# iclavera/learning_to_adapt

Hardware: AMD Instinct MI355X
Metric: controller-steps/sec (n_cand=2000, H=30, ens=5) (higher is better)
Workload: dtype f32

## Files before the change

### learning_to_adapt_amd/csrc/l2a_mfma.h

```cpp
#pragma once

#include <type_traits>

#include "l2a_kernels.h"

#ifndef L2A_XEARLY
#define L2A_XEARLY 1
#endif

#ifndef L2A_NW
#define L2A_NW 4
#endif

typedef unsigned int u32x4 __attribute__((ext_vector_type(4)));
__device__ __forceinline__ __amdgpu_buffer_rsrc_t l2a_rsrc(const void* base, long long bytes) {
    return __builtin_amdgcn_make_buffer_rsrc(const_cast<void*>(base), 0, (int)bytes, 0x00020000);
}
__device__ __forceinline__ f32x4 l2a_ldw(__amdgpu_buffer_rsrc_t rs, int voff, int soff) {
    return __builtin_bit_cast(f32x4, __builtin_amdgcn_raw_buffer_load_b128(rs, voff, soff, 0));
}

template <bool GACT>
__device__ __forceinline__ f32x4 l2a_actv(f32x4 v, int kind, float floor) {
    if (GACT) return l2a_act4(v, kind);
    v.x = l2a_max_nan(v.x, floor); v.y = l2a_max_nan(v.y, floor);
    v.z = l2a_max_nan(v.z, floor); v.w = l2a_max_nan(v.w, floor);
    return v;
}

__device__ __forceinline__ float l2a_sum_xor16(float x) {
    const unsigned int u = __float_as_uint(x);
    const auto r = __builtin_amdgcn_permlane16_swap(u, u, false, false);
    return __uint_as_float(r[0]) + __uint_as_float(r[1]);
}
__device__ __forceinline__ float l2a_sum_xor32(float x) {
    const unsigned int u = __float_as_uint(x);
    const auto r = __builtin_amdgcn_permlane32_swap(u, u, false, false);
    return __uint_as_float(r[0]) + __uint_as_float(r[1]);
}

#define L2A_MFMA4(a, b, c) __builtin_amdgcn_mfma_f32_4x4x1f32((a), (b), (c), 0, 0, 0)

#define L2A_OPAQUE(v) asm volatile("" : "+v"(v))

#ifndef L2A_TIMELINE
#define L2A_TS(slot)
#else
#define L2A_TS(slot)                                                                        \
    if (p.dbg && pairid == 0 && e < 8 && grp < 2) {                                         \
        unsigned long long ts_;                                                             \
        asm volatile("s_memtime %0\n\ts_waitcnt lgkmcnt(0)" : "=s"(ts_) : : "memory");       \
        if (lane == 0) p.dbg[(((long long)(grp * p.h + t) * 8 + e) * 8 + wave) * 16 + (slot)] = ts_; \
    }
#endif

#define L2A_STAGE_MFMA(CA, CB)                                                             \
    _Pragma("unroll") for (int ii = 0; ii < 4; ++ii)                                       \
        _Pragma("unroll") for (int nt = 0; nt < NT; ++nt)                                  \
            _Pragma("unroll") for (int tt = TW - 1; tt >= 0; --tt)    \
                acc[nt][tt] = L2A_MFMA(CA[tt][ii], CB[nt][ii], acc[nt][tt]);

#define L2A_STAGE(CA, CB, FA, FB, SOFF, IMM, GF)                                           \
    {                                                                                      \
        _Pragma("unroll") for (int tt = 0; tt < TW; ++tt)                                  \
            FA[tt] = l2a_ldw(rs, voff[tt] + (IMM), (SOFF));                                \
        _Pragma("unroll") for (int nt = 0; nt < NT; ++nt)                                  \
            FB[nt] = hin[(nt * HT + (GF)) * 64 + lane];                                    \
        L2A_STAGE_MFMA(CA, CB)                                                             \
         \
        __builtin_amdgcn_sched_group_barrier(0x100, NT, 0);                                \
        _Pragma("unroll") for (int tt = 0; tt < TW; ++tt) {                                \
            __builtin_amdgcn_sched_group_barrier(0x008, 4 * NT, 0);                        \
            __builtin_amdgcn_sched_group_barrier(0x020, 1, 0);                             \
        }                                                                                  \
        __builtin_amdgcn_sched_barrier(0);                                                 \
    }

#define L2A_PFT_MAX 6
#define L2A_PFT(TW_, OT_) ((OT_) <= 2 ? ((TW_) < L2A_PFT_MAX ? (TW_) : L2A_PFT_MAX) : ((TW_) < 2 ? (TW_) : 2))

template <int NT, int TW, int TPW, int OT, bool LAST>
__device__ __forceinline__ void l2a_hidden_gemm(__amdgpu_buffer_rsrc_t rs, __amdgpu_buffer_rsrc_t rsn,
                                                const int (&voff)[TPW], const int (&voffn)[TPW], int twn,
                                                int tile0, const f32x4* hin,
                                                f32x4 (&aA)[TPW], f32x4 (&aB)[TPW],
                                                f32x4 (&pfO)[TPW][OT], f32x4 (&acc)[NT][TPW], int lane,
                                                const float* bias_lds, f32x4 (&bias)[TPW], const int (&olane)[OT]) {
    constexpr int HT = L2A_NW * TPW;
    static_assert(HT % 4 == 0, "the k-group pipeline is unrolled by 4");
    f32x4 aC[TW], aD[TW], bA[NT], bB[NT], bC[NT], bD[NT];
#pragma unroll
    for (int nt = 0; nt < NT; ++nt) {
        bA[nt] = hin[(nt * HT + 0) * 64 + lane];
        bB[nt] = hin[(nt * HT + 1) * 64 + lane];
#pragma unroll
        for (int tt = 0; tt < TW; ++tt) acc[nt][tt] = (f32x4){0.f, 0.f, 0.f, 0.f};
    }
#pragma unroll
    for (int nt = 0; nt < NT; ++nt) { L2A_OPAQUE(bA[nt]); L2A_OPAQUE(bB[nt]); }
    __builtin_amdgcn_sched_barrier(0);

#pragma unroll 1
    for (int g = 0; g < HT - 4; g += 4) {
        const int soff = (g + 2) * 1024;
        L2A_STAGE(aA, bA, aC, bC, soff, 0, g + 2)
        L2A_STAGE(aB, bB, aD, bD, soff, 1024, g + 3)
        L2A_STAGE(aC, bC, aA, bA, soff, 2048, g + 4)
        L2A_STAGE(aD, bD, aB, bB, soff, 3072, g + 5)
    }
    L2A_STAGE(aA, bA, aC, bC, (HT - 2) * 1024, 0, HT - 2)
    L2A_STAGE(aB, bB, aD, bD, (HT - 2) * 1024, 1024, HT - 1)
    {
        if (LAST) {
#pragma unroll
            for (int tt = 0; tt < L2A_PFT(TW, OT); ++tt)
#pragma unroll
                for (int c = 0; c < OT; ++c)
                    if (((tt * OT + c) & 1) == 0)
                        pfO[tt][c] = l2a_ldw(rsn, olane[c] + (tile0 + tt) * 1024, c * HT * 1024);
        } else {
#pragma unroll
            for (int tt = 0; tt < TPW; ++tt)
                if (tt < twn) aA[tt] = l2a_ldw(rsn, voffn[tt], 0);
        }
        L2A_STAGE_MFMA(aC, bC)
        __builtin_amdgcn_sched_barrier(0);
    }
    {
#pragma unroll
        for (int tt = 0; tt < TW; ++tt) bias[tt] = *reinterpret_cast<const f32x4*>(bias_lds + 16 * tt);
        if (LAST) {
#pragma unroll
            for (int tt = 0; tt < L2A_PFT(TW, OT); ++tt)
#pragma unroll
                for (int c = 0; c < OT; ++c)
                    if (((tt * OT + c) & 1) == 1)
                        pfO[tt][c] = l2a_ldw(rsn, olane[c] + (tile0 + tt) * 1024, c * HT * 1024);
        } else {
#pragma unroll
            for (int tt = 0; tt < TPW; ++tt)
                if (tt < twn) aB[tt] = l2a_ldw(rsn, voffn[tt] + 1024, 0);
        }
        L2A_STAGE_MFMA(aD, bD)
        __builtin_amdgcn_sched_barrier(0);
    }
}

template <int NT, int TW, int TPW, int OT, int NPF, bool O4, class PF>
__device__ __forceinline__ void l2a_out_phase(const f32x4 (&hreg)[NT][TPW], f32x4 (&pfO)[TPW][OT],
                                              __amdgpu_buffer_rsrc_t rs_out, int tile0, PF prefetch,
                                              f32x4* pbuf, int chunk0, int lane, const int (&olane)[OT]) {
    constexpr int HT = L2A_NW * TPW;
    constexpr int CS = TPW / 2;
    constexpr int NCH = TW / CS;
    f32x4 a[TW][OT];
#pragma unroll
    for (int tt = 0; tt < TW; ++tt)
#pragma unroll
        for (int c = 0; c < OT; ++c)
            a[tt][c] = (tt < L2A_PFT(TW, OT)) ? pfO[tt][c]
                                              : l2a_ldw(rs_out, olane[c] + (tile0 + tt) * 1024, c * HT * 1024);
    prefetch();
    f32x4 acc[NCH][NT][OT];
#pragma unroll
    for (int ch = 0; ch < NCH; ++ch)
#pragma unroll
        for (int nt = 0; nt < NT; ++nt)
#pragma unroll
            for (int c = 0; c < OT; ++c) acc[ch][nt][c] = (f32x4){0.f, 0.f, 0.f, 0.f};
#pragma unroll
    for (int t2 = 0; t2 < CS; ++t2)
#pragma unroll
        for (int ii = 0; ii < 4; ++ii)
#pragma unroll
            for (int ch = 0; ch < NCH; ++ch)
#pragma unroll
                for (int nt = 0; nt < NT; ++nt)
#pragma unroll
                    for (int c = 0; c < OT; ++c)
                        acc[ch][nt][c] = (O4 && c == OT - 1)
                            ? L2A_MFMA4(a[ch * CS + t2][c][ii], hreg[nt][ch * CS + t2][ii], acc[ch][nt][c])
                            : L2A_MFMA(a[ch * CS + t2][c][ii], hreg[nt][ch * CS + t2][ii], acc[ch][nt][c]);
    {
        constexpr int NLATE = (TW - L2A_PFT(TW, OT)) * OT;
        constexpr int NMFMA = TW * 4 * NT * OT;
#pragma unroll
        for (int i = 0; i < NLATE; ++i) {
            __builtin_amdgcn_sched_group_barrier(0x020, 1, 0);
            __builtin_amdgcn_sched_group_barrier(0x008, 2, 0);
        }
        constexpr int PER = (NMFMA - 2 * NLATE) / NPF > 0 ? (NMFMA - 2 * NLATE) / NPF : 1;
#pragma unroll
        for (int i = 0; i < NPF; ++i) {
            __builtin_amdgcn_sched_group_barrier(0x008, PER, 0);
            __builtin_amdgcn_sched_group_barrier(0x020, 1, 0);
        }
    }
#pragma unroll
    for (int nt = 0; nt < NT; ++nt)
#pragma unroll
        for (int c = 0; c < OT; ++c)
            pbuf[((chunk0 * NT + nt) * OT + c) * 64 + lane] = (NCH == 2) ? acc[0][nt][c] + acc[NCH - 1][nt][c] : acc[0][nt][c];
}

template <int NT, int TPW, int OT, int KG0, bool GACT, int K0L = 4, bool N1 = false, bool O4 = false, bool FAN = false, bool WHOLE = false>
__global__ void __launch_bounds__(64 * L2A_NW) l2a_rollout_mfma_k(const L2AKParams p) {
    static_assert(!(FAN && WHOLE), "an instance is general, member fan or whole-tiles-only");
    constexpr bool NOHALF = FAN || WHOLE;
    constexpr int HT = L2A_NW * TPW;
    constexpr int TH = TPW / 2;
    static_assert(TPW % 2 == 0, "half members split a wave's tiles in two");
    constexpr int CST_BOUT = 32 * KG0 + 32 * OT;
    constexpr int CST_BHID = CST_BOUT + 16 * OT;
    constexpr int PS = L2A_NW * NT * OT * 64;
    const int NRM_SET = p.cst_set;
    const int LB = p.lb;
    extern __shared__ __attribute__((aligned(16))) char l2a_smem[];
    f32x4* buf0 = reinterpret_cast<f32x4*>(l2a_smem);
    f32x4* buf1 = buf0 + p.sa_elems;
    f32x4* pbase = buf0 + (LB > 1 ? LB : 2) * p.sa_elems;
    float* nrm = reinterpret_cast<float*>(buf0 + p.cst_off);

    const int tid = threadIdx.x;
    const int lane = tid & 63;
    const int wave = __builtin_amdgcn_readfirstlane(tid >> 6);
    const int jc = lane & 15;
    const int qq = lane >> 4;
    const int c0 = wave * TPW;
    int olane[OT];
#pragma unroll
    for (int c = 0; c < OT; ++c) olane[c] = ((O4 && c == OT - 1) ? ((lane & 48) | (lane & 3)) : lane) * 16;

    const int tail = p.split_from >= 0;
    const int in_tail = tail && (int)blockIdx.x >= p.split_from;
    const int split = FAN ? 3 : WHOLE ? 0 : (tail ? (in_tail ? p.split : 0) : p.split);
    const int n_tiles = p.m * p.tiles_per_env;
    const int n_pairs = tail ? n_tiles - p.split_from : n_tiles;
    int bid, grp, lpair, pairid;
    if (!tail && p.pl_units > 0) {
        const int hx = (int)blockIdx.x & 7, idx = (int)blockIdx.x >> 3;
        const int xcd = hx;
        const int f = p.pl_f, wide = p.pl_r * (f + 1);
        int u, k, xu;
        if (xcd < wide) { u = xcd / (f + 1); k = xcd - u * (f + 1); xu = f + 1; }
// ... 60 lines not shown
        float v;
        if (o < CST_BOUT) v = src[p.nm_off + o];
        else if (o < CST_BHID) v = src[p.pk_bout + (o - CST_BOUT)];
        else {
            const int l = (o - CST_BHID) / (16 * HT);
            v = src[p.raw_b[l] + (o - CST_BHID - l * 16 * HT)];
        }
        nrm[i] = v;
    }

    f32x4 st[NT][OT];
#pragma unroll
    for (int nt = 0; nt < NT; ++nt) {
        const float* orow = p.obs0 + (p.obs_per_row ? (long long)row[nt] : (long long)env) * obs_dim;
#pragma unroll
        for (int c = 0; c < OT; ++c)
#pragma unroll
            for (int ii = 0; ii < 4; ++ii) {
                const int dim = 16 * c + 4 * qq + ii;
                const float v = orow[dim < obs_dim ? dim : obs_dim - 1];
                st[nt][c][ii] = (dim < obs_dim) ? v : 0.0f;
            }
    }
    __syncthreads();

    const int ga0 = obs_dim >> 4;
    f32x4 av_next[NT][2];
    int aoff[NT][2][4];
#pragma unroll
    for (int nt = 0; nt < NT; ++nt)
#pragma unroll
        for (int s = 0; s < 2; ++s)
#pragma unroll
            for (int ii = 0; ii < 4; ++ii) {
                const int ka = 16 * (ga0 + s) + 4 * qq + ii - obs_dim;
                const bool in = (ka >= 0) && (ka < act_dim);
                aoff[nt][s][ii] = in ? (row[nt] * act_dim + ka) * 4 : 0x7ffffff0;
            }
    const long long a_step = (long long)R * act_dim;
    auto load_actions = [&](int t, f32x4 (&dst)[NT][2]) {
        const __amdgpu_buffer_rsrc_t ars = l2a_rsrc(p.actions + (long long)t * a_step, a_step * 4);
#pragma unroll
        for (int nt = 0; nt < NT; ++nt)
#pragma unroll
            for (int s = 0; s < 2; ++s)
#pragma unroll
                for (int ii = 0; ii < 4; ++ii)
                    dst[nt][s][ii] = __builtin_bit_cast(float, __builtin_amdgcn_raw_buffer_load_b32(ars, aoff[nt][s][ii], 0, 0));
    };
    f32x4 av[NT][2];
    float asq[NT];
    auto take_actions = [&](int t_fetch) {
#pragma unroll
        for (int nt = 0; nt < NT; ++nt) {
            av[nt][0] = av_next[nt][0];
            av[nt][1] = av_next[nt][1];
            float s = 0.0f;
#pragma unroll
            for (int ii = 0; ii < 4; ++ii) {
                s = fmaf(av[nt][0][ii], av[nt][0][ii], s);
                s = fmaf(av[nt][1][ii], av[nt][1][ii], s);
            }
            asq[nt] = s;
        }
        load_actions((t_fetch < p.h) ? t_fetch : p.h - 1, av_next);
    };
    load_actions(0, av_next);
    take_actions(1);

    float ret[NT];
#pragma unroll
    for (int nt = 0; nt < NT; ++nt) ret[nt] = p.ret_in ? p.ret_in[(long long)env * p.n + (valid[nt] ? cand[nt] : p.c_hi - 1)] : 0.0f;

    f32x4* hcur = buf0;
    f32x4* hoth = buf1;
    const float e_count = (float)e_loop;
    const float e_inv = 1.0f / e_count;
    double disc_pow = p.disc0;
    unsigned int spin_left = p.spin_limit;
    const unsigned int xtag0 = p.xtag;
    const __amdgpu_buffer_rsrc_t xrs = l2a_rsrc(p.xbuf, FAN ? (long long)n_pairs * e_loop * 2 * (NT * OT * 2 * 64 * 16)
                                                        : split ? (long long)n_pairs * 8 * (NT * OT * 2 * 64 * 16) : 16);

    constexpr int KG0P = (FAN && KG0 <= 2) ? KG0 : 1;
    f32x4 pfL0[KG0P][TPW];
    f32x4 pfA[TPW], pfB[TPW];
    f32x4 pfO[TPW][OT];
    int voff[TPW], voffh[TPW], voff0[TPW];
    const int tile0h = grp * (HT / 2) + wave * TH;
#pragma unroll
    for (int tt = 0; tt < TPW; ++tt) {
        voff[tt] = lane * 16 + (c0 + tt) * HT * 1024;
        voffh[tt] = lane * 16 + (tile0h + (tt < TH ? tt : 0)) * HT * 1024;
        voff0[tt] = lane * 16 + (c0 + tt) * KG0 * 1024;
    }
    const long long w0_bytes = (long long)HT * KG0 * 1024, wm_bytes = (long long)HT * HT * 1024,
                    wo_bytes = (long long)OT * HT * 1024;
    {
        const __amdgpu_buffer_rsrc_t r0 = l2a_rsrc(set_base(seq(0)) + p.pk_w0, w0_bytes);
#pragma unroll
        for (int g = 0; g < KG0P; ++g)
#pragma unroll
            for (int tt = 0; tt < TPW; ++tt) pfL0[g][tt] = l2a_ldw(r0, voff0[tt] + g * 1024, 0);
    }

    for (int t = 0; t < p.h; ++t) {
        f32x4 dsum[NT][OT], dgrp[NT][OT], qsh[NT][OT];
#pragma unroll
        for (int nt = 0; nt < NT; ++nt)
#pragma unroll
            for (int c = 0; c < OT; ++c) {
                dsum[nt][c] = (f32x4){0.f, 0.f, 0.f, 0.f};
                dgrp[nt][c] = (f32x4){0.f, 0.f, 0.f, 0.f};
                qsh[nt][c] = (f32x4){0.f, 0.f, 0.f, 0.f};
            }

        const unsigned int xtag = xtag0 + (unsigned int)(t + 1);
        constexpr int XREG = NT * OT * 2 * 64 * 16;
        auto xbase = [&](int g, int region) { return (((lpair * 2 + g) * 2 + (t & 1)) * 2 + region) * XREG + lane * 16; };
        auto xput = [&](int region, const f32x4 (&v)[NT][OT]) {
#pragma unroll
            for (int nt = 0; nt < NT; ++nt)
#pragma unroll
                for (int c = 0; c < OT; ++c)
#pragma unroll
                    for (int hh = 0; hh < 2; ++hh) {
                        u32x4 g;
                        g.x = xtag; g.y = __float_as_uint(v[nt][c][2 * hh]);
                        g.z = xtag; g.w = __float_as_uint(v[nt][c][2 * hh + 1]);
                        __builtin_amdgcn_raw_buffer_store_b128(g, xrs, xbase(grp, region) + ((nt * OT + c) * 2 + hh) * 1024, 0, L2A_SC1);
                    }
        };
        auto xget = [&](int region, f32x4 (&v)[NT][OT]) {
            bool ok = true;
#pragma unroll
            for (int nt = 0; nt < NT; ++nt)
#pragma unroll
                for (int c = 0; c < OT; ++c)
#pragma unroll
                    for (int hh = 0; hh < 2; ++hh) {
                        const u32x4 g = __builtin_amdgcn_raw_buffer_load_b128(
                            xrs, xbase(grp ^ 1, region) + ((nt * OT + c) * 2 + hh) * 1024, 0, L2A_SC1);
                        v[nt][c][2 * hh] = __uint_as_float(g.y);
                        v[nt][c][2 * hh + 1] = __uint_as_float(g.w);
                        ok = ok && (g.x == xtag) && (g.z == xtag);
                    }
            return ok;
        };

        bool xearly = false;
        u32x4 sw[2][NT][OT][2];
        for (int b0 = 0; b0 < n_seq; b0 += LB) {
            const int nb = (n_seq - b0 < LB) ? n_seq - b0 : LB;
            f32x4 hreg[NT][TPW];

            auto layer0 = [&](int j, auto last_tag) {
                constexpr bool last_l0 = decltype(last_tag)::value;
                const int i = b0 + j;
                const int e = seq(i);
                const float* wb = set_base(e);
                const float* nr = nrm + i * NRM_SET;
                const __amdgpu_buffer_rsrc_t rs_out = l2a_rsrc(wb + p.pk_wout, wo_bytes);
                L2A_TS(0)
                const __amdgpu_buffer_rsrc_t r0 = l2a_rsrc(wb + p.pk_w0, w0_bytes);
                f32x4 a[KG0][TPW];
#pragma unroll
                for (int g = 0; g < KG0; ++g)
#pragma unroll
                    for (int tt = 0; tt < TPW; ++tt)
                        a[g][tt] = (g < KG0P) ? pfL0[g < KG0P ? g : 0][tt] : l2a_ldw(r0, voff0[tt] + g * 1024, 0);
                L2A_TS(8)
                constexpr bool XPRE = (KG0 <= 2);
                auto norm_in = [&](int g, const f32x4& mu, const f32x4& iv, f32x4 (&x)[NT]) {
#pragma unroll
                    for (int nt = 0; nt < NT; ++nt) {
                        f32x4 sv = (f32x4){0.f, 0.f, 0.f, 0.f};
                        if (g < OT) sv = st[nt][g < OT ? g : 0];
                        f32x4 aa = (f32x4){0.f, 0.f, 0.f, 0.f};
                        if (g == ga0) aa = av[nt][0];
                        if (g == ga0 + 1) aa = av[nt][1];
#pragma unroll
                        for (int ii = 0; ii < 4; ++ii) x[nt][ii] = ((sv[ii] + aa[ii]) - mu[ii]) * iv[ii];
                    }
                };
                f32x4 xin[XPRE ? KG0 : 1][NT];
                if (XPRE) {
                    f32x4 mu[KG0], iv[KG0];
#pragma unroll
                    for (int g = 0; g < KG0; ++g) {
                        mu[g] = *reinterpret_cast<const f32x4*>(nr + 16 * g + 4 * qq);
                        iv[g] = *reinterpret_cast<const f32x4*>(nr + 16 * KG0 + 16 * g + 4 * qq);
                    }
                    __builtin_amdgcn_sched_barrier(0);
#pragma unroll
                    for (int g = 0; g < KG0; ++g) norm_in(g, mu[g], iv[g], xin[XPRE ? g : 0]);
                }
                f32x4 bias0[TPW];
#pragma unroll
                for (int tt = 0; tt < TPW; ++tt)
                    bias0[tt] = *reinterpret_cast<const f32x4*>(nr + CST_BHID + 16 * (c0 + tt) + 4 * qq);
                f32x4 acc[NT][TPW];
                auto l0_mfma = [&](auto npf_tag) {
                    constexpr int NPF = decltype(npf_tag)::value;
#pragma unroll
                    for (int nt = 0; nt < NT; ++nt)
#pragma unroll
                        for (int tt = 0; tt < TPW; ++tt) acc[nt][tt] = (f32x4){0.f, 0.f, 0.f, 0.f};
#pragma unroll
                    for (int g = 0; g < KG0; ++g) {
                        f32x4 xg[NT];
                        if (XPRE) {
#pragma unroll
                            for (int nt = 0; nt < NT; ++nt) xg[nt] = xin[XPRE ? g : 0][nt];
                        } else {
                            const f32x4 mu = *reinterpret_cast<const f32x4*>(nr + 16 * g + 4 * qq);
                            const f32x4 iv = *reinterpret_cast<const f32x4*>(nr + 16 * KG0 + 16 * g + 4 * qq);
                            norm_in(g, mu, iv, xg);
                        }
#pragma unroll
                        for (int ii = 0; ii < 4; ++ii) {
                            if (g == KG0 - 1 && ii >= K0L) continue;
#pragma unroll
                            for (int nt = 0; nt < NT; ++nt)
#pragma unroll
                                for (int tt = 0; tt < TPW; ++tt)
                                    acc[nt][tt] = L2A_MFMA(a[g][tt][ii], xg[nt][ii], acc[nt][tt]);
                        }
                    }
                    constexpr int NM = ((KG0 - 1) * 4 + K0L) * NT * TPW;
                    constexpr int PER = NM / (NPF > 0 ? NPF : 1) > 0 ? NM / (NPF > 0 ? NPF : 1) : 1;
                    __builtin_amdgcn_sched_group_barrier(0x020, (KG0 - KG0P) * TPW, 0);
#pragma unroll
                    for (int k = 0; k < NPF; ++k) {
                        __builtin_amdgcn_sched_group_barrier(0x008, PER, 0);
                        __builtin_amdgcn_sched_group_barrier(0x020, 1, 0);
                    }
                };
                if (N1) {
#pragma unroll
                    for (int tt = 0; tt < L2A_PFT(TPW, OT); ++tt)
#pragma unroll
                        for (int c = 0; c < OT; ++c)
                            pfO[tt][c] = l2a_ldw(rs_out, olane[c] + (c0 + tt) * 1024, c * HT * 1024);
                    l0_mfma(std::integral_constant<int, L2A_PFT(TPW, OT) * OT>{});
                } else if (!last_l0) {
                    const __amdgpu_buffer_rsrc_t r0n = l2a_rsrc(set_base(seq(i + 1)) + p.pk_w0, w0_bytes);
#pragma unroll
                    for (int g = 0; g < KG0P; ++g)
#pragma unroll
                        for (int tt = 0; tt < TPW; ++tt) pfL0[g][tt] = l2a_ldw(r0n, voff0[tt] + g * 1024, 0);
                    l0_mfma(std::integral_constant<int, KG0P * TPW>{});
                } else {
                    const int e0 = seq(b0);
                    const __amdgpu_buffer_rsrc_t rs1 = l2a_rsrc(set_base(e0) + p.pk_wmid, wm_bytes);
                    const bool next_half = !NOHALF && (e0 == e_shared) && n_hidden == 2;
                    if (next_half) {
#pragma unroll
                        for (int tt = 0; tt < TH; ++tt) {
                            pfA[tt] = l2a_ldw(rs1, voffh[tt], 0);
                            pfB[tt] = l2a_ldw(rs1, voffh[tt] + 1024, 0);
                        }
                        l0_mfma(std::integral_constant<int, 2 * TH>{});
                    } else {
#pragma unroll
                        for (int tt = 0; tt < TPW; ++tt) {
                            pfA[tt] = l2a_ldw(rs1, voff[tt], 0);
                            pfB[tt] = l2a_ldw(rs1, voff[tt] + 1024, 0);
                        }
                        l0_mfma(std::integral_constant<int, 2 * TPW>{});
                    }
                }
                L2A_TS(9)
#pragma unroll
                for (int tt = 0; tt < TPW; ++tt) {
#pragma unroll
                    for (int nt = 0; nt < NT; ++nt)
                        hreg[nt][tt] = l2a_actv<GACT>(acc[nt][tt] + bias0[tt], p.hidden_act, p.hid_floor);
                }
                L2A_TS(10)
                if (!N1) {
                    f32x4* hdst = (LB > 1) ? buf0 + j * p.sa_elems : hcur;
#pragma unroll
                    for (int tt = 0; tt < TPW; ++tt)
#pragma unroll
                        for (int nt = 0; nt < NT; ++nt) hdst[(nt * HT + c0 + tt) * 64 + lane] = hreg[nt][tt];
                }
                L2A_TS(1)
            };

            auto member = [&](int j, auto last_tag) {
                constexpr bool last_set = decltype(last_tag)::value;
                const int i = b0 + j;
                const int e = seq(i);
                const bool is_half = !NOHALF && last_set && (e == e_shared);
                const float* wb = set_base(e);
                const float* nr = nrm + i * NRM_SET;
                const __amdgpu_buffer_rsrc_t rs_out = l2a_rsrc(wb + p.pk_wout, wo_bytes);
                f32x4* pb = (LB > 1) ? pbase + j * PS : hoth;
                L2A_TS(2)
                if (!N1) {
                    f32x4 acc[NT][TPW], bias[TPW];
                    for (int l = 1; last_set && l < n_hidden - 1; ++l) {
                        const float* wl = wb + p.pk_wmid + (long long)(l - 1) * p.pk_wmid_stride;
                        const bool next_half = is_half && (l == n_hidden - 2);
                        l2a_hidden_gemm<NT, TPW, TPW, OT, false>(l2a_rsrc(wl, wm_bytes), l2a_rsrc(wl + p.pk_wmid_stride, wm_bytes),
                                                                 voff, next_half ? voffh : voff, next_half ? TH : TPW, 0,
                                                                 hcur, pfA, pfB, pfO, acc, lane,
                                                                 nr + CST_BHID + l * (16 * HT) + 16 * c0 + 4 * qq, bias, olane);
#pragma unroll
                        for (int tt = 0; tt < TPW; ++tt) {
#pragma unroll
                            for (int nt = 0; nt < NT; ++nt)
                                hoth[(nt * HT + c0 + tt) * 64 + lane] = l2a_actv<GACT>(acc[nt][tt] + bias[tt], p.hidden_act, p.hid_floor);
                        }
                        __syncthreads();
                        f32x4* tmp = hcur; hcur = hoth; hoth = tmp;
                    }
                    if (LB == 1) pb = hoth;
                    L2A_TS(15)
                    const f32x4* hin = (LB > 1) ? buf0 + j * p.sa_elems : hcur;
                    const __amdgpu_buffer_rsrc_t rs_last =
                        l2a_rsrc(wb + p.pk_wmid + (long long)(n_hidden - 2) * p.pk_wmid_stride, wm_bytes);
                    const float* bl = nr + CST_BHID + (n_hidden - 1) * (16 * HT);
                    if (!is_half) {
                        l2a_hidden_gemm<NT, TPW, TPW, OT, true>(rs_last, rs_out, voff, voff, TPW, c0, hin, pfA, pfB, pfO,
                                                                acc, lane, bl + 16 * c0 + 4 * qq, bias, olane);
#pragma unroll
                        for (int tt = 0; tt < TPW; ++tt) {
#pragma unroll
                            for (int nt = 0; nt < NT; ++nt)
                                hreg[nt][tt] = l2a_actv<GACT>(acc[nt][tt] + bias[tt], p.hidden_act, p.hid_floor);
                        }
                    } else {
                        l2a_hidden_gemm<NT, TH, TPW, OT, true>(rs_last, rs_out, voffh, voffh, TH, tile0h, hin, pfA, pfB,
                                                               pfO, acc, lane, bl + 16 * tile0h + 4 * qq, bias, olane);
#pragma unroll
                        for (int tt = 0; tt < TH; ++tt) {
#pragma unroll
                            for (int nt = 0; nt < NT; ++nt)
                                hreg[nt][tt] = l2a_actv<GACT>(acc[nt][tt] + bias[tt], p.hidden_act, p.hid_floor);
                        }
                    }
                }
                L2A_TS(3)
                if (last_set) {
                    const __amdgpu_buffer_rsrc_t r0n = l2a_rsrc(set_base(seq((i + 1 < n_seq) ? i + 1 : 0)) + p.pk_w0, w0_bytes);
                    auto pf_l0 = [&]() {
#pragma unroll
                        for (int g = 0; g < KG0P; ++g)
#pragma unroll
                            for (int tt = 0; tt < TPW; ++tt) pfL0[g][tt] = l2a_ldw(r0n, voff0[tt] + g * 1024, 0);
                    };
                    if (is_half) l2a_out_phase<NT, TH, TPW, OT, KG0P * TPW, O4>(hreg, pfO, rs_out, tile0h, pf_l0, pb, wave, lane, olane);
                    else l2a_out_phase<NT, TPW, TPW, OT, KG0P * TPW, O4>(hreg, pfO, rs_out, c0, pf_l0, pb, wave, lane, olane);
                } else {
                    const int en = seq(i + 1);
                    const __amdgpu_buffer_rsrc_t rsn = l2a_rsrc(set_base(en) + p.pk_wmid, wm_bytes);
                    if (!NOHALF && en == e_shared) {
                        l2a_out_phase<NT, TPW, TPW, OT, 2 * TH, O4>(hreg, pfO, rs_out, c0, [&]() {
#pragma unroll
                            for (int tt = 0; tt < TH; ++tt) {
                                pfA[tt] = l2a_ldw(rsn, voffh[tt], 0);
                                pfB[tt] = l2a_ldw(rsn, voffh[tt] + 1024, 0);
                            }
                        }, pb, wave, lane, olane);
                    } else {
                        l2a_out_phase<NT, TPW, TPW, OT, 2 * TPW, O4>(hreg, pfO, rs_out, c0, [&]() {
#pragma unroll
                            for (int tt = 0; tt < TPW; ++tt) {
                                pfA[tt] = l2a_ldw(rsn, voff[tt], 0);
                                pfB[tt] = l2a_ldw(rsn, voff[tt] + 1024, 0);
                            }
                        }, pb, wave, lane, olane);
                    }
                }
                L2A_TS(4)
            };
            for (int j = 0; j + 1 < nb; ++j) layer0(j, std::false_type{});
            layer0(nb - 1, std::true_type{});
            if (!N1) __syncthreads();
            for (int j = 0; j + 1 < nb; ++j) member(j, std::false_type{});
            member(nb - 1, std::true_type{});

            __syncthreads();
            constexpr bool XE_OK = L2A_XEARLY && !NOHALF && NT == 1 && OT <= 2 && KG0 <= 2;
            const bool xe = XE_OK && split == 2 && nb >= 2 && b0 + nb == n_seq;
            for (int jj = 0; jj < nb; ++jj) {
                const int j = (xe && wave == 0) ? (jj == 0 ? nb - 1 : jj - 1) : jj;
                const int i = b0 + j;
                const int e = seq(i);
                const bool is_half = !NOHALF && (e == e_shared);
                const float* nr = nrm + i * NRM_SET;
                const f32x4* pb = (LB > 1) ? pbase + j * PS : hoth;
                L2A_TS(5)
                if (e == e_half && !split) {
#pragma unroll
                    for (int nt = 0; nt < NT; ++nt)
#pragma unroll
                        for (int c = 0; c < OT; ++c) {
                            dsum[nt][c] = dgrp[nt][c];
                            dgrp[nt][c] = (f32x4){0.f, 0.f, 0.f, 0.f};
                        }
                }
#pragma unroll
                for (int c = 0; c < OT; ++c) {
                    f32x4 part[L2A_NW][NT];
#pragma unroll
                    for (int ch = 0; ch < L2A_NW; ++ch)
#pragma unroll
                        for (int nt = 0; nt < NT; ++nt) part[ch][nt] = pb[((ch * NT + nt) * OT + c) * 64 + lane];
                    const f32x4 bias = *reinterpret_cast<const f32x4*>(nr + CST_BOUT + 16 * c + 4 * qq);
                    const f32x4 omu = *reinterpret_cast<const f32x4*>(nr + 32 * KG0 + 16 * c + 4 * qq);
                    const f32x4 osd = *reinterpret_cast<const f32x4*>(nr + 32 * KG0 + 16 * OT + 16 * c + 4 * qq);
                    __builtin_amdgcn_sched_barrier(0);
#pragma unroll
                    for (int nt = 0; nt < NT; ++nt) {
                        static_assert(L2A_NW == 4, "the canonical tree below is written out for four waves");
                        f32x4 s = (part[0][nt] + part[1][nt]) + (part[2][nt] + part[3][nt]);
                        if (is_half) {
                            qsh[nt][c] = s;
                        } else {
                            if (O4 && c == OT - 1) {
#pragma unroll
                                for (int ii = 0; ii < 4; ++ii) s[ii] = l2a_sum_xor32(l2a_sum_xor16(s[ii]));
                            }
                            s = l2a_actv<GACT>(s + bias, p.output_act, p.out_floor);
                            if (FAN) dgrp[nt][c] = s * osd + omu;
                            else dgrp[nt][c] += s * osd + omu;
                        }
                    }
                }
                if (!NOHALF && split == 2 && i == n_full - 1 && wave == (XE_OK ? 1 : 0)) xput(0, dgrp);
                if (xe && wave == 0 && jj == 0) xput(1, qsh);
                if (xe && wave == 3 && jj == nb - 1) {
#pragma unroll
                    for (int r = 0; r < 2; ++r)
#pragma unroll
                        for (int nt = 0; nt < NT; ++nt)
#pragma unroll
                            for (int c = 0; c < OT; ++c)
#pragma unroll
                                for (int hh = 0; hh < 2; ++hh)
                                    sw[r][nt][c][hh] = (r == 1 || e_loop > 1)
                                        ? __builtin_amdgcn_raw_buffer_load_b128(xrs, xbase(grp ^ 1, r) + ((nt * OT + c) * 2 + hh) * 1024, 0, L2A_SC1)
                                        : (u32x4){xtag, 0u, xtag, 0u};
                }
                L2A_TS(6)
            }
            if (xe) xearly = true;
            if (N1) { f32x4* tmp = hcur; hcur = hoth; hoth = tmp; }
        }

        { const int e = 7; L2A_TS(9) }
        float asq_t[NT];
#pragma unroll
        for (int nt = 0; nt < NT; ++nt) asq_t[nt] = asq[nt];
        if (FAN) {
            constexpr int XREGF = NT * OT * 2 * 64 * 16;
            auto fbase = [&](int g) { return ((lpair * e_loop + g) * 2 + (t & 1)) * XREGF + lane * 16; };
            if (wave == 0) {
#pragma unroll
                for (int nt = 0; nt < NT; ++nt)
#pragma unroll
                    for (int c = 0; c < OT; ++c) {
#pragma unroll
                        for (int hh = 0; hh < 2; ++hh) {
                            u32x4 g;
                            g.x = xtag; g.y = __float_as_uint(dgrp[nt][c][2 * hh]);
                            g.z = xtag; g.w = __float_as_uint(dgrp[nt][c][2 * hh + 1]);
                            __builtin_amdgcn_raw_buffer_store_b128(g, xrs, fbase(grp) + ((nt * OT + c) * 2 + hh) * 1024, 0, L2A_SC1);
                        }
                        xlds[((grp * NT + nt) * OT + c) * 64 + lane] = dgrp[nt][c];
                    }
            }
            { const int e = 7; L2A_TS(11) }
            take_actions(t + 2);
            for (int k = wave; k < e_loop - 1; k += L2A_NW) {
                int g2 = grp + 1 + k;
                if (g2 >= e_loop) g2 -= e_loop;
                f32x4 oth[NT][OT];
                while (true) {
                    bool ok = true;
#pragma unroll
                    for (int nt = 0; nt < NT; ++nt)
#pragma unroll
                        for (int c = 0; c < OT; ++c)
#pragma unroll
                            for (int hh = 0; hh < 2; ++hh) {
                                const u32x4 g = __builtin_amdgcn_raw_buffer_load_b128(
                                    xrs, fbase(g2) + ((nt * OT + c) * 2 + hh) * 1024, 0, L2A_SC1);
                                oth[nt][c][2 * hh] = __uint_as_float(g.y);
                                oth[nt][c][2 * hh + 1] = __uint_as_float(g.w);
                                ok = ok && (g.x == xtag) && (g.z == xtag);
                            }
                    if (__all(ok)) break;
                    if (spin_left == 0) {
                        if (lane == 0) __hip_atomic_fetch_or(p.status, 1u, __ATOMIC_RELAXED, __HIP_MEMORY_SCOPE_SYSTEM);
                        break;
                    }
                    --spin_left;
                    __builtin_amdgcn_s_sleep(4);
                }
#pragma unroll
                for (int nt = 0; nt < NT; ++nt)
#pragma unroll
                    for (int c = 0; c < OT; ++c) xlds[((g2 * NT + nt) * OT + c) * 64 + lane] = oth[nt][c];
            }
            { const int e = 7; L2A_TS(12) }
            __syncthreads();
            { const int e = 7; L2A_TS(13) }
#pragma unroll
            for (int nt = 0; nt < NT; ++nt)
#pragma unroll
                for (int c = 0; c < OT; ++c) {
                    dsum[nt][c] = (f32x4){0.f, 0.f, 0.f, 0.f};
                    dgrp[nt][c] = (f32x4){0.f, 0.f, 0.f, 0.f};
                }
            {
                constexpr int EMAX = 8;
                f32x4 v[EMAX][NT][OT];
#pragma unroll
                for (int e = 0; e < EMAX; ++e) {
                    const int es = e < e_loop ? e : e_loop - 1;
#pragma unroll
                    for (int nt = 0; nt < NT; ++nt)
#pragma unroll
                        for (int c = 0; c < OT; ++c) v[e][nt][c] = xlds[((es * NT + nt) * OT + c) * 64 + lane];
                }
                __builtin_amdgcn_sched_barrier(0);
#pragma unroll
                for (int e = 0; e < EMAX; ++e)
#pragma unroll
                    for (int nt = 0; nt < NT; ++nt)
#pragma unroll
// ... 228 lines not shown
```

Baseline: 702.7.

## Move per-tile weight offsets into scalar registers and specialize final reduction batch

Replaces the per-tile VGPR offset arrays (voff, voffh, voff0) with one lane16 vector offset plus wave-uniform scalar bases, so buffer loads carry the tile stride in the SGPR soffset field. This frees vector registers and address arithmetic in the hot hidden-GEMM loop. The per-batch reduction phase becomes a lambda specialized at compile time for the last batch, so the half and early-exchange branches drop out of non-final batches. It also enables a register-prefetch layer-0 schedule for the non-FAN case. The risks are higher SGPR pressure and a different instruction schedule.

New measurement: 712.8, median of 6. 1.4% higher.

```diff
diff --git a/learning_to_adapt_amd/csrc/l2a_mfma.h b/learning_to_adapt_amd/csrc/l2a_mfma.h
--- a/learning_to_adapt_amd/csrc/l2a_mfma.h
+++ b/learning_to_adapt_amd/csrc/l2a_mfma.h
@@ -42,6 +42,7 @@
 #define L2A_MFMA4(a, b, c) __builtin_amdgcn_mfma_f32_4x4x1f32((a), (b), (c), 0, 0, 0)
 
 #define L2A_OPAQUE(v) asm volatile("" : "+v"(v))
+#define L2A_OPAQUE_S(v) asm("" : "+s"(v))
 
 #ifndef L2A_TIMELINE
 #define L2A_TS(slot)
@@ -60,31 +61,40 @@
             _Pragma("unroll") for (int tt = TW - 1; tt >= 0; --tt)    \
                 acc[nt][tt] = L2A_MFMA(CA[tt][ii], CB[nt][ii], acc[nt][tt]);
 
+#define L2A_STAGE_REST(CA, CB, FB, GF, NA)                                                 \
+        _Pragma("unroll") for (int nt = 0; nt < NT; ++nt)                                  \
+            FB[nt] = hin[(nt * HT + (GF)) * 64 + lane];                                    \
+        L2A_STAGE_MFMA(CA, CB)                                                             \
+        __builtin_amdgcn_sched_group_barrier(0x100, NT, 0);                                \
+        _Pragma("unroll") for (int tt = 0; tt < (NA); ++tt) {                              \
+            __builtin_amdgcn_sched_group_barrier(0x008, 4 * NT, 0);                        \
+            __builtin_amdgcn_sched_group_barrier(0x020, 1, 0);                             \
+        }                                                                                  \
+        __builtin_amdgcn_sched_barrier(0);
+
 #define L2A_STAGE(CA, CB, FA, FB, SOFF, IMM, GF)                                           \
     {                                                                                      \
         _Pragma("unroll") for (int tt = 0; tt < TW; ++tt)                                  \
             FA[tt] = l2a_ldw(rs, voff[tt] + (IMM), (SOFF));                                \
-        _Pragma("unroll") for (int nt = 0; nt < NT; ++nt)                                  \
-            FB[nt] = hin[(nt * HT + (GF)) * 64 + lane];                                    \
-        L2A_STAGE_MFMA(CA, CB)                                                             \
-         \
-        __builtin_amdgcn_sched_group_barrier(0x100, NT, 0);                                \
-        _Pragma("unroll") for (int tt = 0; tt < TW; ++tt) {                                \
-            __builtin_amdgcn_sched_group_barrier(0x008, 4 * NT, 0);                        \
-            __builtin_amdgcn_sched_group_barrier(0x020, 1, 0);                             \
-        }                                                                                  \
-        __builtin_amdgcn_sched_barrier(0);                                                 \
-    }
-
+        L2A_STAGE_REST(CA, CB, FB, GF, TW)                                                 \
+    }
+#define L2A_STAGE_S(CA, CB, FA, FB, SOFF, IMM, GF)                                         \
+    {                                                                                      \
+        int so_ = sb + (SOFF);                                                             \
+        L2A_OPAQUE_S(so_);                                                                 \
+        _Pragma("unroll") for (int tt = 0; tt < TW; ++tt)                                  \
+            FA[tt] = l2a_ldw(rs, lane16 + (IMM), so_ + tt * (HT * 1024));                  \
+        L2A_STAGE_REST(CA, CB, FB, GF, TW)                                                 \
+    }
 #define L2A_PFT_MAX 6
 #define L2A_PFT(TW_, OT_) ((OT_) <= 2 ? ((TW_) < L2A_PFT_MAX ? (TW_) : L2A_PFT_MAX) : ((TW_) < 2 ? (TW_) : 2))
 
 template <int NT, int TW, int TPW, int OT, bool LAST>
 __device__ __forceinline__ void l2a_hidden_gemm(__amdgpu_buffer_rsrc_t rs, __amdgpu_buffer_rsrc_t rsn,
-                                                const int (&voff)[TPW], const int (&voffn)[TPW], int twn,
+                                                int sb, int sbn, int twn,
                                                 int tile0, const f32x4* hin,
                                                 f32x4 (&aA)[TPW], f32x4 (&aB)[TPW],
-                                                f32x4 (&pfO)[TPW][OT], f32x4 (&acc)[NT][TPW], int lane,
+                                                f32x4 (&pfO)[TPW][OT], f32x4 (&acc)[NT][TPW], int lane, int lane16,
                                                 const float* bias_lds, f32x4 (&bias)[TPW], const int (&olane)[OT]) {
     constexpr int HT = L2A_NW * TPW;
     static_assert(HT % 4 == 0, "the k-group pipeline is unrolled by 4");
@@ -103,25 +113,27 @@
 #pragma unroll 1
     for (int g = 0; g < HT - 4; g += 4) {
         const int soff = (g + 2) * 1024;
-        L2A_STAGE(aA, bA, aC, bC, soff, 0, g + 2)
-        L2A_STAGE(aB, bB, aD, bD, soff, 1024, g + 3)
-        L2A_STAGE(aC, bC, aA, bA, soff, 2048, g + 4)
-        L2A_STAGE(aD, bD, aB, bB, soff, 3072, g + 5)
-    }
-    L2A_STAGE(aA, bA, aC, bC, (HT - 2) * 1024, 0, HT - 2)
-    L2A_STAGE(aB, bB, aD, bD, (HT - 2) * 1024, 1024, HT - 1)
+        L2A_STAGE_S(aA, bA, aC, bC, soff, 0, g + 2)
+        L2A_STAGE_S(aB, bB, aD, bD, soff, 1024, g + 3)
+        L2A_STAGE_S(aC, bC, aA, bA, soff, 2048, g + 4)
+        L2A_STAGE_S(aD, bD, aB, bB, soff, 3072, g + 5)
+    }
+    L2A_STAGE_S(aA, bA, aC, bC, (HT - 2) * 1024, 0, HT - 2)
+    L2A_STAGE_S(aB, bB, aD, bD, (HT - 2) * 1024, 1024, HT - 1)
     {
+        int so_ = LAST ? tile0 * 1024 : sbn;
+        L2A_OPAQUE_S(so_);
         if (LAST) {
 #pragma unroll
             for (int tt = 0; tt < L2A_PFT(TW, OT); ++tt)
 #pragma unroll
                 for (int c = 0; c < OT; ++c)
                     if (((tt * OT + c) & 1) == 0)
-                        pfO[tt][c] = l2a_ldw(rsn, olane[c] + (tile0 + tt) * 1024, c * HT * 1024);
+                        pfO[tt][c] = l2a_ldw(rsn, olane[c], so_ + (tt + c * HT) * 1024);
         } else {
 #pragma unroll
             for (int tt = 0; tt < TPW; ++tt)
-                if (tt < twn) aA[tt] = l2a_ldw(rsn, voffn[tt], 0);
+                if (tt < twn) aA[tt] = l2a_ldw(rsn, lane16, so_ + tt * (HT * 1024));
         }
         L2A_STAGE_MFMA(aC, bC)
         __builtin_amdgcn_sched_barrier(0);
@@ -129,17 +141,19 @@
     {
 #pragma unroll
         for (int tt = 0; tt < TW; ++tt) bias[tt] = *reinterpret_cast<const f32x4*>(bias_lds + 16 * tt);
+        int so_ = LAST ? tile0 * 1024 : sbn;
+        L2A_OPAQUE_S(so_);
         if (LAST) {
 #pragma unroll
             for (int tt = 0; tt < L2A_PFT(TW, OT); ++tt)
 #pragma unroll
                 for (int c = 0; c < OT; ++c)
                     if (((tt * OT + c) & 1) == 1)
-                        pfO[tt][c] = l2a_ldw(rsn, olane[c] + (tile0 + tt) * 1024, c * HT * 1024);
+                        pfO[tt][c] = l2a_ldw(rsn, olane[c], so_ + (tt + c * HT) * 1024);
         } else {
 #pragma unroll
             for (int tt = 0; tt < TPW; ++tt)
-                if (tt < twn) aB[tt] = l2a_ldw(rsn, voffn[tt] + 1024, 0);
+                if (tt < twn) aB[tt] = l2a_ldw(rsn, lane16 + 1024, so_ + tt * (HT * 1024));
         }
         L2A_STAGE_MFMA(aD, bD)
         __builtin_amdgcn_sched_barrier(0);
@@ -154,12 +168,14 @@
     constexpr int CS = TPW / 2;
     constexpr int NCH = TW / CS;
     f32x4 a[TW][OT];
+    int so_ = tile0 * 1024;
+    L2A_OPAQUE_S(so_);
 #pragma unroll
     for (int tt = 0; tt < TW; ++tt)
 #pragma unroll
         for (int c = 0; c < OT; ++c)
             a[tt][c] = (tt < L2A_PFT(TW, OT)) ? pfO[tt][c]
-                                              : l2a_ldw(rs_out, olane[c] + (tile0 + tt) * 1024, c * HT * 1024);
+                                              : l2a_ldw(rs_out, olane[c], so_ + (tt + c * HT) * 1024);
     prefetch();
     f32x4 acc[NCH][NT][OT];
 #pragma unroll
@@ -386,18 +402,15 @@
     const __amdgpu_buffer_rsrc_t xrs = l2a_rsrc(p.xbuf, FAN ? (long long)n_pairs * e_loop * 2 * (NT * OT * 2 * 64 * 16)
                                                         : split ? (long long)n_pairs * 8 * (NT * OT * 2 * 64 * 16) : 16);
 
-    constexpr int KG0P = (FAN && KG0 <= 2) ? KG0 : 1;
+    constexpr int KG0P = (KG0 <= 2) ? KG0 : 1;
+    constexpr bool L0RF = !FAN && KG0P == KG0;
     f32x4 pfL0[KG0P][TPW];
     f32x4 pfA[TPW], pfB[TPW];
     f32x4 pfO[TPW][OT];
-    int voff[TPW], voffh[TPW], voff0[TPW];
-    const int tile0h = grp * (HT / 2) + wave * TH;
-#pragma unroll
-    for (int tt = 0; tt < TPW; ++tt) {
-        voff[tt] = lane * 16 + (c0 + tt) * HT * 1024;
-        voffh[tt] = lane * 16 + (tile0h + (tt < TH ? tt : 0)) * HT * 1024;
-        voff0[tt] = lane * 16 + (c0 + tt) * KG0 * 1024;
-    }
+    const int lane16 = lane * 16;
+    const int tile0h = __builtin_amdgcn_readfirstlane(grp * (HT / 2) + wave * TH);
+    const int sbf = c0 * (HT * 1024), sbh = tile0h * (HT * 1024), sb0 = c0 * (KG0 * 1024);
+    auto sbase = [](int v) { L2A_OPAQUE_S(v); return v; };
     const long long w0_bytes = (long long)HT * KG0 * 1024, wm_bytes = (long long)HT * HT * 1024,
                     wo_bytes = (long long)OT * HT * 1024;
     {
@@ -405,18 +418,17 @@
 #pragma unroll
         for (int g = 0; g < KG0P; ++g)
 #pragma unroll
-            for (int tt = 0; tt < TPW; ++tt) pfL0[g][tt] = l2a_ldw(r0, voff0[tt] + g * 1024, 0);
+            for (int tt = 0; tt < TPW; ++tt) pfL0[g][tt] = l2a_ldw(r0, lane16, sb0 + (tt * KG0 + g) * 1024);
     }
 
     for (int t = 0; t < p.h; ++t) {
-        f32x4 dsum[NT][OT], dgrp[NT][OT], qsh[NT][OT];
+        f32x4 dsum[NT][OT], dgrp[NT][OT];
 #pragma unroll
         for (int nt = 0; nt < NT; ++nt)
 #pragma unroll
             for (int c = 0; c < OT; ++c) {
                 dsum[nt][c] = (f32x4){0.f, 0.f, 0.f, 0.f};
                 dgrp[nt][c] = (f32x4){0.f, 0.f, 0.f, 0.f};
-                qsh[nt][c] = (f32x4){0.f, 0.f, 0.f, 0.f};
             }
 
         const unsigned int xtag = xtag0 + (unsigned int)(t + 1);
@@ -452,10 +464,83 @@
             return ok;
         };
 
-        bool xearly = false;
+        f32x4 qsh[NT][OT];
         u32x4 sw[2][NT][OT][2];
-        for (int b0 = 0; b0 < n_seq; b0 += LB) {
-            const int nb = (n_seq - b0 < LB) ? n_seq - b0 : LB;
+#pragma unroll
+        for (int nt = 0; nt < NT; ++nt)
+#pragma unroll
+            for (int c = 0; c < OT; ++c) qsh[nt][c] = (f32x4){0.f, 0.f, 0.f, 0.f};
+        int b0 = 0, nb;
+        auto phase_c = [&](auto last_tag) {
+            constexpr bool last_batch = decltype(last_tag)::value;
+            constexpr bool XE_OK = L2A_XEARLY && !NOHALF && NT == 1 && OT <= 2 && KG0 <= 2;
+            const bool xe = last_batch && XE_OK && split == 2 && nb >= 2;
+            for (int jj = 0; jj < nb; ++jj) {
+                const int j = (xe && wave == 0) ? (jj == 0 ? nb - 1 : jj - 1) : jj;
+                const int i = b0 + j;
+                const int e = seq(i);
+                const bool is_half = last_batch && !NOHALF && (e == e_shared);
+                const float* nr = nrm + i * NRM_SET;
+                const f32x4* pb = (LB > 1) ? pbase + j * PS : hoth;
+                L2A_TS(5)
+                if (e == e_half && !split) {
+#pragma unroll
+                    for (int nt = 0; nt < NT; ++nt)
+#pragma unroll
+                        for (int c = 0; c < OT; ++c) {
+                            dsum[nt][c] = dgrp[nt][c];
+                            dgrp[nt][c] = (f32x4){0.f, 0.f, 0.f, 0.f};
+                        }
+                }
+#pragma unroll
+                for (int c = 0; c < OT; ++c) {
+                    f32x4 part[L2A_NW][NT];
+#pragma unroll
+                    for (int ch = 0; ch < L2A_NW; ++ch)
+#pragma unroll
+                        for (int nt = 0; nt < NT; ++nt) part[ch][nt] = pb[((ch * NT + nt) * OT + c) * 64 + lane];
+                    const f32x4 bias = *reinterpret_cast<const f32x4*>(nr + CST_BOUT + 16 * c + 4 * qq);
+                    const f32x4 omu = *reinterpret_cast<const f32x4*>(nr + 32 * KG0 + 16 * c + 4 * qq);
+                    const f32x4 osd = *reinterpret_cast<const f32x4*>(nr + 32 * KG0 + 16 * OT + 16 * c + 4 * qq);
+                    __builtin_amdgcn_sched_barrier(0);
+#pragma unroll
+                    for (int nt = 0; nt < NT; ++nt) {
+                        static_assert(L2A_NW == 4, "the canonical tree below is written out for four waves");
+                        f32x4 s = (part[0][nt] + part[1][nt]) + (part[2][nt] + part[3][nt]);
+                        if (is_half) {
+                            qsh[nt][c] = s;
+                        } else {
+                            if (O4 && c == OT - 1) {
+#pragma unroll
+                                for (int ii = 0; ii < 4; ++ii) s[ii] = l2a_sum_xor32(l2a_sum_xor16(s[ii]));
+                            }
+                            s = l2a_actv<GACT>(s + bias, p.output_act, p.out_floor);
+                            if (FAN) dgrp[nt][c] = s * osd + omu;
+                            else dgrp[nt][c] += s * osd + omu;
+                        }
+                    }
+                }
+                if (!NOHALF && split == 2 && i == n_full - 1 && wave == (XE_OK ? 1 : 0)) xput(0, dgrp);
+                if (xe && wave == 0 && jj == 0) xput(1, qsh);
+                if (xe && wave == 3 && jj == nb - 1) {
+#pragma unroll
+                    for (int r = 0; r < 2; ++r)
+#pragma unroll
+                        for (int nt = 0; nt < NT; ++nt)
+#pragma unroll
+                            for (int c = 0; c < OT; ++c)
+#pragma unroll
+                                for (int hh = 0; hh < 2; ++hh)
+                                    sw[r][nt][c][hh] = (r == 1 || e_loop > 1)
+                                        ? __builtin_amdgcn_raw_buffer_load_b128(xrs, xbase(grp ^ 1, r) + ((nt * OT + c) * 2 + hh) * 1024, 0, L2A_SC1)
+                                        : (u32x4){xtag, 0u, xtag, 0u};
+                }
+                L2A_TS(6)
+            }
+            return xe;
+        };
+        for (;; b0 += LB) {
+            nb = (n_seq - b0 < LB) ? n_seq - b0 : LB;
             f32x4 hreg[NT][TPW];
 
             auto layer0 = [&](int j, auto last_tag) {
@@ -468,11 +553,12 @@
                 L2A_TS(0)
                 const __amdgpu_buffer_rsrc_t r0 = l2a_rsrc(wb + p.pk_w0, w0_bytes);
                 f32x4 a[KG0][TPW];
+                const int s0 = sbase(sb0);
 #pragma unroll
                 for (int g = 0; g < KG0; ++g)
 #pragma unroll
                     for (int tt = 0; tt < TPW; ++tt)
-                        a[g][tt] = (g < KG0P) ? pfL0[g < KG0P ? g : 0][tt] : l2a_ldw(r0, voff0[tt] + g * 1024, 0);
+                        a[g][tt] = (g < KG0P) ? pfL0[g < KG0P ? g : 0][tt] : l2a_ldw(r0, lane16, s0 + (tt * KG0 + g) * 1024);
                 L2A_TS(8)
                 constexpr bool XPRE = (KG0 <= 2);
                 auto norm_in = [&](int g, const f32x4& mu, const f32x4& iv, f32x4 (&x)[NT]) {
@@ -531,6 +617,21 @@
                                     acc[nt][tt] = L2A_MFMA(a[g][tt][ii], xg[nt][ii], acc[nt][tt]);
                         }
                     }
+                    if constexpr (NPF < 0) {
+                        __builtin_amdgcn_sched_group_barrier(0x008, (KG0 > 1 ? 4 : K0L) * NT * TPW, 0);
+#pragma unroll
+                        for (int k = 0; k < (KG0 - 2) * TPW; ++k) {
+                            __builtin_amdgcn_sched_group_barrier(0x020, 1, 0);
+                            __builtin_amdgcn_sched_group_barrier(0x008, 4 * NT, 0);
+                        }
+#pragma unroll
+                        for (int k = 0; k < (KG0 > 1 ? TPW : 0); ++k) {
+                            __builtin_amdgcn_sched_group_barrier(0x020, 1, 0);
+                            __builtin_amdgcn_sched_group_barrier(0x008, K0L * NT, 0);
+                        }
+                        __builtin_amdgcn_sched_group_barrier(0x020, TPW, 0);
+                        return;
+                    }
                     constexpr int NM = ((KG0 - 1) * 4 + K0L) * NT * TPW;
                     constexpr int PER = NM / (NPF > 0 ? NPF : 1) > 0 ? NM / (NPF > 0 ? NPF : 1) : 1;
                     __builtin_amdgcn_sched_group_barrier(0x020, (KG0 - KG0P) * TPW, 0);
@@ -541,35 +642,38 @@
                     }
                 };
                 if (N1) {
+                    const int so = sbase(c0 * 1024);
 #pragma unroll
                     for (int tt = 0; tt < L2A_PFT(TPW, OT); ++tt)
 #pragma unroll
                         for (int c = 0; c < OT; ++c)
-                            pfO[tt][c] = l2a_ldw(rs_out, olane[c] + (c0 + tt) * 1024, c * HT * 1024);
+                            pfO[tt][c] = l2a_ldw(rs_out, olane[c], so + (tt + c * HT) * 1024);
                     l0_mfma(std::integral_constant<int, L2A_PFT(TPW, OT) * OT>{});
                 } else if (!last_l0) {
                     const __amdgpu_buffer_rsrc_t r0n = l2a_rsrc(set_base(seq(i + 1)) + p.pk_w0, w0_bytes);
+                    if (L0RF) l0_mfma(std::integral_constant<int, -1>{});
 #pragma unroll
                     for (int g = 0; g < KG0P; ++g)
 #pragma unroll
-                        for (int tt = 0; tt < TPW; ++tt) pfL0[g][tt] = l2a_ldw(r0n, voff0[tt] + g * 1024, 0);
-                    l0_mfma(std::integral_constant<int, KG0P * TPW>{});
+                        for (int tt = 0; tt < TPW; ++tt) pfL0[g][tt] = l2a_ldw(r0n, lane16, s0 + (tt * KG0 + g) * 1024);
+                    if (!L0RF) l0_mfma(std::integral_constant<int, KG0P * TPW>{});
                 } else {
                     const int e0 = seq(b0);
                     const __amdgpu_buffer_rsrc_t rs1 = l2a_rsrc(set_base(e0) + p.pk_wmid, wm_bytes);
                     const bool next_half = !NOHALF && (e0 == e_shared) && n_hidden == 2;
+                    const int s1 = sbase(next_half ? sbh : sbf);
                     if (next_half) {
 #pragma unroll
                         for (int tt = 0; tt < TH; ++tt) {
-                            pfA[tt] = l2a_ldw(rs1, voffh[tt], 0);
-                            pfB[tt] = l2a_ldw(rs1, voffh[tt] + 1024, 0);
+                            pfA[tt] = l2a_ldw(rs1, lane16, s1 + tt * (HT * 1024));
+                            pfB[tt] = l2a_ldw(rs1, lane16 + 1024, s1 + tt * (HT * 1024));
                         }
                         l0_mfma(std::integral_constant<int, 2 * TH>{});
                     } else {
 #pragma unroll
                         for (int tt = 0; tt < TPW; ++tt) {
-                            pfA[tt] = l2a_ldw(rs1, voff[tt], 0);
-                            pfB[tt] = l2a_ldw(rs1, voff[tt] + 1024, 0);
+                            pfA[tt] = l2a_ldw(rs1, lane16, s1 + tt * (HT * 1024));
+                            pfB[tt] = l2a_ldw(rs1, lane16 + 1024, s1 + tt * (HT * 1024));
                         }
                         l0_mfma(std::integral_constant<int, 2 * TPW>{});
                     }
@@ -608,8 +712,8 @@
                         const float* wl = wb + p.pk_wmid + (long long)(l - 1) * p.pk_wmid_stride;
                         const bool next_half = is_half && (l == n_hidden - 2);
                         l2a_hidden_gemm<NT, TPW, TPW, OT, false>(l2a_rsrc(wl, wm_bytes), l2a_rsrc(wl + p.pk_wmid_stride, wm_bytes),
-                                                                 voff, next_half ? voffh : voff, next_half ? TH : TPW, 0,
-                                                                 hcur, pfA, pfB, pfO, acc, lane,
+                                                                 sbf, next_half ? sbh : sbf, next_half ? TH : TPW, 0,
+                                                                 hcur, pfA, pfB, pfO, acc, lane, lane16,
                                                                  nr + CST_BHID + l * (16 * HT) + 16 * c0 + 4 * qq, bias, olane);
 #pragma unroll
                         for (int tt = 0; tt < TPW; ++tt) {
@@ -627,8 +731,8 @@
                         l2a_rsrc(wb + p.pk_wmid + (long long)(n_hidden - 2) * p.pk_wmid_stride, wm_bytes);
                     const float* bl = nr + CST_BHID + (n_hidden - 1) * (16 * HT);
                     if (!is_half) {
-                        l2a_hidden_gemm<NT, TPW, TPW, OT, true>(rs_last, rs_out, voff, voff, TPW, c0, hin, pfA, pfB, pfO,
-                                                                acc, lane, bl + 16 * c0 + 4 * qq, bias, olane);
+                        l2a_hidden_gemm<NT, TPW, TPW, OT, true>(rs_last, rs_out, sbf, sbf, TPW, c0, hin, pfA, pfB, pfO,
+                                                                acc, lane, lane16, bl + 16 * c0 + 4 * qq, bias, olane);
 #pragma unroll
                         for (int tt = 0; tt < TPW; ++tt) {
 #pragma unroll
@@ -636,8 +740,8 @@
                                 hreg[nt][tt] = l2a_actv<GACT>(acc[nt][tt] + bias[tt], p.hidden_act, p.hid_floor);
                         }
                     } else {
-                        l2a_hidden_gemm<NT, TH, TPW, OT, true>(rs_last, rs_out, voffh, voffh, TH, tile0h, hin, pfA, pfB,
-                                                               pfO, acc, lane, bl + 16 * tile0h + 4 * qq, bias, olane);
+                        l2a_hidden_gemm<NT, TH, TPW, OT, true>(rs_last, rs_out, sbh, sbh, TH, tile0h, hin, pfA, pfB,
+                                                               pfO, acc, lane, lane16, bl + 16 * tile0h + 4 * qq, bias, olane);
 #pragma unroll
                         for (int tt = 0; tt < TH; ++tt) {
 #pragma unroll
@@ -650,10 +754,11 @@
                 if (last_set) {
                     const __amdgpu_buffer_rsrc_t r0n = l2a_rsrc(set_base(seq((i + 1 < n_seq) ? i + 1 : 0)) + p.pk_w0, w0_bytes);
                     auto pf_l0 = [&]() {
+                        const int s0 = sbase(sb0);
 #pragma unroll
                         for (int g = 0; g < KG0P; ++g)
 #pragma unroll
-                            for (int tt = 0; tt < TPW; ++tt) pfL0[g][tt] = l2a_ldw(r0n, voff0[tt] + g * 1024, 0);
+                            for (int tt = 0; tt < TPW; ++tt) pfL0[g][tt] = l2a_ldw(r0n, lane16, s0 + (tt * KG0 + g) * 1024);
                     };
                     if (is_half) l2a_out_phase<NT, TH, TPW, OT, KG0P * TPW, O4>(hreg, pfO, rs_out, tile0h, pf_l0, pb, wave, lane, olane);
                     else l2a_out_phase<NT, TPW, TPW, OT, KG0P * TPW, O4>(hreg, pfO, rs_out, c0, pf_l0, pb, wave, lane, olane);
@@ -662,18 +767,20 @@
                     const __amdgpu_buffer_rsrc_t rsn = l2a_rsrc(set_base(en) + p.pk_wmid, wm_bytes);
                     if (!NOHALF && en == e_shared) {
                         l2a_out_phase<NT, TPW, TPW, OT, 2 * TH, O4>(hreg, pfO, rs_out, c0, [&]() {
+                            const int s1 = sbase(sbh);
 #pragma unroll
                             for (int tt = 0; tt < TH; ++tt) {
-                                pfA[tt] = l2a_ldw(rsn, voffh[tt], 0);
-                                pfB[tt] = l2a_ldw(rsn, voffh[tt] + 1024, 0);
+                                pfA[tt] = l2a_ldw(rsn, lane16, s1 + tt * (HT * 1024));
+                                pfB[tt] = l2a_ldw(rsn, lane16 + 1024, s1 + tt * (HT * 1024));
                             }
                         }, pb, wave, lane, olane);
                     } else {
                         l2a_out_phase<NT, TPW, TPW, OT, 2 * TPW, O4>(hreg, pfO, rs_out, c0, [&]() {
+                            const int s1 = sbase(sbf);
 #pragma unroll
                             for (int tt = 0; tt < TPW; ++tt) {
-                                pfA[tt] = l2a_ldw(rsn, voff[tt], 0);
-                                pfB[tt] = l2a_ldw(rsn, voff[tt] + 1024, 0);
+                                pfA[tt] = l2a_ldw(rsn, lane16, s1 + tt * (HT * 1024));
+                                pfB[tt] = l2a_ldw(rsn, lane16 + 1024, s1 + tt * (HT * 1024));
                             }
                         }, pb, wave, lane, olane);
                     }
@@ -687,73 +794,12 @@
             member(nb - 1, std::true_type{});
 
             __syncthreads();
-            constexpr bool XE_OK = L2A_XEARLY && !NOHALF && NT == 1 && OT <= 2 && KG0 <= 2;
-            const bool xe = XE_OK && split == 2 && nb >= 2 && b0 + nb == n_seq;
-            for (int jj = 0; jj < nb; ++jj) {
-                const int j = (xe && wave == 0) ? (jj == 0 ? nb - 1 : jj - 1) : jj;
-                const int i = b0 + j;
-                const int e = seq(i);
-                const bool is_half = !NOHALF && (e == e_shared);
-                const float* nr = nrm + i * NRM_SET;
-                const f32x4* pb = (LB > 1) ? pbase + j * PS : hoth;
-                L2A_TS(5)
-                if (e == e_half && !split) {
-#pragma unroll
-                    for (int nt = 0; nt < NT; ++nt)
-#pragma unroll
-                        for (int c = 0; c < OT; ++c) {
-                            dsum[nt][c] = dgrp[nt][c];
-                            dgrp[nt][c] = (f32x4){0.f, 0.f, 0.f, 0.f};
-                        }
-                }
-#pragma unroll
-                for (int c = 0; c < OT; ++c) {
-                    f32x4 part[L2A_NW][NT];
-#pragma unroll
-                    for (int ch = 0; ch < L2A_NW; ++ch)
-#pragma unroll
-                        for (int nt = 0; nt < NT; ++nt) part[ch][nt] = pb[((ch * NT + nt) * OT + c) * 64 + lane];
-                    const f32x4 bias = *reinterpret_cast<const f32x4*>(nr + CST_BOUT + 16 * c + 4 * qq);
-                    const f32x4 omu = *reinterpret_cast<const f32x4*>(nr + 32 * KG0 + 16 * c + 4 * qq);
-                    const f32x4 osd = *reinterpret_cast<const f32x4*>(nr + 32 * KG0 + 16 * OT + 16 * c + 4 * qq);
-                    __builtin_amdgcn_sched_barrier(0);
-#pragma unroll
-                    for (int nt = 0; nt < NT; ++nt) {
-                        static_assert(L2A_NW == 4, "the canonical tree below is written out for four waves");
-                        f32x4 s = (part[0][nt] + part[1][nt]) + (part[2][nt] + part[3][nt]);
-                        if (is_half) {
-                            qsh[nt][c] = s;
-                        } else {
-                            if (O4 && c == OT - 1) {
-#pragma unroll
-                                for (int ii = 0; ii < 4; ++ii) s[ii] = l2a_sum_xor32(l2a_sum_xor16(s[ii]));
-                            }
-                            s = l2a_actv<GACT>(s + bias, p.output_act, p.out_floor);
-                            if (FAN) dgrp[nt][c] = s * osd + omu;
-                            else dgrp[nt][c] += s * osd + omu;
-                        }
-                    }
-                }
-                if (!NOHALF && split == 2 && i == n_full - 1 && wave == (XE_OK ? 1 : 0)) xput(0, dgrp);
-                if (xe && wave == 0 && jj == 0) xput(1, qsh);
-                if (xe && wave == 3 && jj == nb - 1) {
-#pragma unroll
-                    for (int r = 0; r < 2; ++r)
-#pragma unroll
-                        for (int nt = 0; nt < NT; ++nt)
-#pragma unroll
-                            for (int c = 0; c < OT; ++c)
-#pragma unroll
-                                for (int hh = 0; hh < 2; ++hh)
-                                    sw[r][nt][c][hh] = (r == 1 || e_loop > 1)
-                                        ? __builtin_amdgcn_raw_buffer_load_b128(xrs, xbase(grp ^ 1, r) + ((nt * OT + c) * 2 + hh) * 1024, 0, L2A_SC1)
-                                        : (u32x4){xtag, 0u, xtag, 0u};
-                }
-                L2A_TS(6)
-            }
-            if (xe) xearly = true;
+            if (b0 + nb >= n_seq) break;
+            phase_c(std::false_type{});
             if (N1) { f32x4* tmp = hcur; hcur = hoth; hoth = tmp; }
         }
+        const bool xearly = phase_c(std::true_type{});
+        if (N1) { f32x4* tmp = hcur; hcur = hoth; hoth = tmp; }
 
         { const int e = 7; L2A_TS(9) }
         float asq_t[NT];
```
